# Zhengjun-Du/LC-CRF-SLAM

Hardware: AMD Instinct MI355X
Metric: CRF mean-field iters/sec (higher is better)
Workload: dtype f32; 1 GPU; C2: 2000 keypoints, 5 iters, two 2-D kernels (TUM3.yaml), L=2; frames_in_flight_per_gpu=16384, handles=1, distinct_frames=64, n_points=2000, n_iters=5, n_labels=2, engine=fused

## Files before the change

### lc-crf-slam_amd/csrc/engine.h

```cpp
#pragma once

#include <hip/hip_runtime.h>
#include <stdint.h>

#include <stdlib.h>

#include "../../include/lccrf.h"

#ifndef LCCRF_INSTRUMENT
#define LCCRF_INSTRUMENT 0
#endif

namespace lccrf {

#if LCCRF_INSTRUMENT
inline const char *ab_env(const char *name) { return getenv(name); }
#else
inline const char *ab_env(const char *) { return nullptr; }
#endif

constexpr int kMaxD = LCCRF_MAX_DIMS;
constexpr int kEmpty = -1;

constexpr int kNdistAxes = 4;
// ... 177 lines not shown
    c.nontemporal = c.alone_32bit > 0 && p.nontemporal;
    return p;
}

constexpr int kSortPlan = 3 * kMaxD + 2;
struct SortScratch {
    int bits;
    int rm_points;
    int *cells;
    int *partial;
    int *plan;
    int *code;
    int *hist;
    int *start;
    int *tiles;
    int *perm, *iperm;
    int vcap;
    int vbits;
    unsigned long long *vcode;
    unsigned long long *vkey;
    int *vph;
    int *vbad;
    int *vhist, *vstart;
    int *vtiles;
    int *vpartial;
    long long *vplan;
};

void launch_sort_points(const KernelDev &kd, const CrfDev &c, const SortScratch &ss, hipStream_t s);
void launch_permute_rows(const CrfDev &c, float *dst, const float *src, int width, int gather, hipStream_t s);
void launch_build_kernel(const KernelDev &kd, const CrfDev &c, hipStream_t s, const SortScratch *vsort, int *bstat);
void launch_norm(const KernelDev &kd, const CrfDev &c, int maxV, hipStream_t s);
struct UnaryTable { float v[2 * LCCRF_MAX_LABELS + 1]; };
void launch_unary_from_label_tbl(const CrfDev &c, const int16_t *label, const UnaryTable &tbl, hipStream_t s);
void launch_start(const CrfDev &c, hipStream_t s);
void launch_step_stream(const CrfDev &c, const KernelDev *kds, const int *maxV, float relax,
                        hipStream_t s, const float *const *compat = nullptr, const float *const *pre = nullptr);
void launch_norm_factor(const CrfDev &c, const float *norm, float *out, int root, hipStream_t s);
void launch_splat_scaled(const KernelDev &kd, const float *in, int in_stride, int L, int F, int maxV, const float *pre, hipStream_t s);
void launch_map(const CrfDev &c, hipStream_t s);
void launch_map_of(const CrfDev &c, const float *prob, int16_t *map, hipStream_t s);
void launch_exp_and_normalize(const CrfDev &c, const float *in, float *out, float scale, float relax, hipStream_t s);
void launch_step_init(const CrfDev &c, float *out, hipStream_t s);
void launch_filter(const KernelDev &kd, const CrfDev &c, int maxV, const float *in, float *out, int accumulate, hipStream_t s,
                   int reverse = 0, const float **blurred = nullptr, const float *compat = nullptr, const float *pre = nullptr);
const float *launch_filter_values1(const KernelDev &kd, const CrfDev &c, int maxV, const float *in, int in_stride, hipStream_t s,
                                   int reverse);
hipError_t time_blur_pass(const KernelDev &kd, int F, int maxV, int L, int reps, hipStream_t s, float *ms_per_launch);
enum { kStageCopy = 0, kStagePosition = 1, kStageImageU8 = 2, kStageImageF32 = 3 };
void launch_stage_features(float *dst, const void *src, int n, int d, int mode, int width, float posdev, float featuredev,
                           hipStream_t s);
void launch_validate_npoints(const int *in, int *out, int F, int maxN, int *bad, hipStream_t s);

struct BackwardRequest {
    int T;
    float relax;
    const float *grad_prob;
    float *grad_unary;
    float *grad_weights;
    float *const *grad_features;
    float *grad_compat;
    bool compat_form;
    float *grad_model;
    const int *counts;
};
struct BackwardArea {
    size_t slice;
// ... 54 lines not shown
inline int copy_matrices(const TermModel &t, int K, float (*mu)[4])
{
    int has_mu = 0;
    for (int k = 0; k < K; ++k)
        if (t.mats && t.mats[k]) {
            has_mu |= 1 << k;
            for (int e = 0; e < 4; ++e) mu[k][e] = t.mats[k][e];
        }
    return has_mu;
}
struct ConvergeOut {
    int *iterations;
    float *delta;
    int *changed;
    int *converged;
};

bool build_small_supported(const KernelDev *kds, int n, int max_points);
void launch_build_small(const KernelDev *kds, int n, int max_points, const CrfDev &c, hipStream_t s);

bool slam_shaped(const CrfDev &c, const KernelDev *kds, bool u16_tables);
bool fused_supported(const CrfDev &c, const KernelDev *kds, const int *maxV, const int *maxRow,
                     size_t *lds_bytes);
struct LeanPrep {
    unsigned char *buf = nullptr;
    size_t bytes = 0;
    bool valid = false, timed = false;
    unsigned long long key = 0, seen_key = 0;
    unsigned runs = 0;
    hipEvent_t ev0 = nullptr, ev1 = nullptr;
};
size_t lean_prep_bytes(const CrfDev &c, const KernelDev *kds, const int *maxV, const int *maxRow);
inline int fused_report(int lanes, int ppt, int chain0) { return lanes | ppt << 16 | (chain0 ? 1 << 20 : 0); }
struct SizedRequest {
    Schedule run;
    TermModel terms;
    ConvergeOut out;
    LeanPrep *prep;
};
struct SizedLaunch {
    int report;
    int shape;
};
SizedLaunch launch_inference(const CrfDev &c, const KernelDev *kds, const int *maxV, const int *maxRow, const SizedRequest &rq,
                             hipStream_t s);

struct ConvergeTrack {
    float *prev;
    unsigned *acc;
    int *done;
    int *running;
    ConvergeOut out;
};
void launch_track_begin(const CrfDev &c, const ConvergeTrack &tk, int max_iter, hipStream_t s);
void launch_track_step(const CrfDev &c, const ConvergeTrack &tk, int t, int max_iter, int criterion, float tol, hipStream_t s);
void launch_track_restore(const CrfDev &c, const ConvergeTrack &tk, int t_last, hipStream_t s);

bool frame_supported(const CrfDev &c, const KernelDev *kds);
struct FrameRequest {
    Schedule run;
    TermModel terms;
    int *status;
    int *frame_status;
    const int16_t *label;
    const float *tbl5;
    unsigned *done;
    unsigned done_epoch;
    ConvergeOut out;
    bool allow_small;
    unsigned *dual;
    unsigned dual_epoch;
// ... 24 lines not shown
```

### lc-crf-slam_amd/csrc/fused_engine.hip

```cpp
#include "engine.h"
#include "device_math.h"
#include "fused_loop.h"
#include "fused_lean.h"
#include "fused_variant.h"
#include "dispatch.h"

#include <algorithm>
#include <cstdio>
#include <cstdlib>

namespace lccrf {

namespace {

using namespace fl;

constexpr int kPrepMinFrames = 64;

struct FusedArgs {
    KernelDev kd[kMaxFusedK];
    FusedLayout lay;
    int n_iter, with_map;
    float relax, omr;
    long long *timing;
    int timing_block, timing_lane;
    int dbg;
    unsigned char *prep;
    int prep_stride;
    int Vcap[kMaxFusedK];
};

template <int NT, int PPT, int K, int CH, int MODE>
__global__ void __launch_bounds__(NT, 4) k_fused(CrfDev c, FusedArgs a)
{
    constexpr int D1 = kD1;
    extern __shared__ __attribute__((aligned(16))) unsigned char smem[];
    const int f = blockIdx.x;
// ... 503 lines not shown
    for (int k = 0; k < c.K; ++k) a.Vcap[k] = maxV[k];
    const LeanPrepPlan pp = lean_prep_plan(a.lay, c.K, a.Vcap, sh.nt, sh.ppt, sh.lean);
    static const bool no_prep = ab_env("LCCRF_NO_LEAN_PREP") != nullptr;
    int mode = 0;
    const int pieces = (sh.lean ? 1 : 2) * sh.nt * 16;
    bool pieces_ok = true;
    for (int k = 0; k < c.K; ++k) pieces_ok = pieces_ok && pp.row_bytes[k] <= pieces && pp.nbr_bytes[k] <= pieces;
    if (prep && prep->buf && !no_prep && pieces_ok && c.F >= kPrepMinFrames && (size_t)pp.total * (size_t)c.F <= prep->bytes) {
        unsigned long long key = 1469598103934665603ull;
        auto mix = [&](const void *p, size_t n) { for (size_t i = 0; i < n; ++i) key = (key ^ static_cast<const unsigned char *>(p)[i]) * 1099511628211ull; };
        mix(&a.lay, sizeof(a.lay));
        mix(a.Vcap, sizeof(int) * c.K);
        const int shape[6] = {c.F, c.K, sh.ppt, sh.points, sh.nt, sh.lean ? 2 : sh.small ? 1 : 0};
        mix(shape, sizeof(shape));
        mix(&kLeanPrepFormat, sizeof(kLeanPrepFormat));
        mix(&pp, sizeof(pp));
        a.prep = prep->buf;
        a.prep_stride = pp.total;
        if (prep->valid && prep->key == key) {
            mode = 2;
        } else if (prep->seen_key == key) {
            if (prep->ev0) (void)hipEventRecord(prep->ev0, s);
            launch_shape(c, a, s, 1, sh);
            if (prep->ev1) (void)hipEventRecord(prep->ev1, s);
            prep->timed = prep->ev0 && prep->ev1;
            prep->valid = true;
            prep->key = key;
            ++prep->runs;
            mode = 2;
        } else {
            prep->seen_key = key;
        }
    }
    launch_shape(c, a, s, mode, sh);
    stamps.print(s);
    return SizedLaunch{fused_report(sh.nt, sh.ppt, a.lay.chain0), sh.report()};
}

}
```

### lc-crf-slam_amd/csrc/fused_lean.h

```cpp
#pragma once

#include "fused_loop.h"

#ifndef LCCRF_LEAN_SKIP
#define LCCRF_LEAN_SKIP 0
#endif
#define LEAN_SKIP(bit) ((LCCRF_LEAN_SKIP & (bit)) != 0)

namespace lccrf {
namespace fl {

#ifndef LCCRF_CHAIN_TOP
#define LCCRF_CHAIN_TOP 16
#endif
constexpr int kLeanChainTop = LCCRF_CHAIN_TOP;
static_assert(kLeanChainTop == kChainTop || kLeanChainTop == 32, "16 rows on the lanes chain_top_rank names, or a full wavefront");
constexpr int kLeanMaxRounds = 4;
__host__ __device__ constexpr int lean_rounds(int nt) { return nt >= 512 ? 3 : 4; }
__host__ __device__ constexpr int lean_max_v(int nt) { return 3 * (nt - 64); }

__host__ __device__ inline int lean_plane_floats(int NA, int V0)
{
    const int top = V0 < kLeanChainTop ? V0 : kLeanChainTop;
    return (NA * kD1 + 11 * top + 3 * (V0 - top) + 16 + 63) & ~63;
// ... 390 lines not shown
    }
    for (int j = 0; j < kD1; ++j) {
        for (int v = tid; v < Vk; v += NT) {
            const unsigned n = gnbr[(size_t)j * Epad + v], n1 = n & 0xffffu, n2 = n >> 16;
            out[j * axis_words + perm[v]] = (n1 ? (unsigned)perm[n1 - 1] + 1u : 0u) | ((n2 ? (unsigned)perm[n2 - 1] + 1u : 0u) << 16);
        }
    }
    __syncthreads();
    for (int v = tid; v <= Vk; v += NT) row[v] = nrow[v];
    __syncthreads();
}

typedef unsigned lean_u3 __attribute__((ext_vector_type(3)));
struct LeanSrc {
    __amdgpu_buffer_rsrc_t nbr[kMaxFusedK];
    __amdgpu_buffer_rsrc_t bary[kMaxFusedK];
    __amdgpu_buffer_rsrc_t norm[kMaxFusedK];
    __amdgpu_buffer_rsrc_t unary;
    int nbr_axis_bytes[kMaxFusedK];
    int off_nbr[kMaxFusedK], off_bary[kMaxFusedK], off_norm[kMaxFusedK], off_unary;
};
constexpr int kLeanRecPoints = 4 * kNTSmall;
constexpr int kLeanRecUnary = 0;
constexpr int kLeanRecBary = kLeanRecUnary + kLeanRecPoints * 8;
constexpr int kLeanRecNorm = kLeanRecBary + kMaxFusedK * kLeanRecPoints * kD1 * 4;
constexpr int kLeanRecNbr = kLeanRecNorm + kMaxFusedK * kLeanRecPoints * 4;
constexpr int kLeanRecNbrAxis = lean_max_v(kNTSmall) * 4;
constexpr int kLeanRecBytes = (kLeanRecNbr + kD1 * kLeanRecNbrAxis + 255) & ~255;
__device__ __forceinline__ __amdgpu_buffer_rsrc_t lean_rsrc(const void *p, size_t bytes)
{
    return __builtin_amdgcn_make_buffer_rsrc(const_cast<void *>(p), 0, (int)bytes, 0x00020000);
}

template <int PPT, int K>
__device__ __forceinline__ void opaque_ids(PointRegs<PPT, K> &pr)
{
#pragma unroll
    for (int s = 0; s < PPT; ++s) {
#pragma unroll
        for (int k = 0; k < K; ++k) asm volatile("" : "+v"(pr.ix[s][k][0]), "+v"(pr.ix[s][k][1]), "+v"(pr.ix[s][k][2]));
    }
}

struct LeanPrepPlan {
    int cl_off;
    int row_off[kMaxFusedK], row_bytes[kMaxFusedK];
    int nbr_off[kMaxFusedK], nbr_bytes[kMaxFusedK];
    int snbr_off[kMaxFusedK], snbr_axis[kMaxFusedK];
    int total;
};
constexpr unsigned kLeanPrepFormat = 8;
__host__ __device__ inline LeanPrepPlan lean_prep_plan(const FusedLayout &lay, int K, const int *Vcap, int nt, int ppt, bool sorted = false)
{
    LeanPrepPlan p{};
    int o = K * ppt * nt * 12;
    p.cl_off = o;
    o += nt * 8;
    for (int k = 0; k < K; ++k) {
        p.row_off[k] = o;
        p.row_bytes[k] = ((Vcap[k] + 2) * 2 + 15) & ~15;
        o += p.row_bytes[k];
        p.nbr_off[k] = o;
        p.nbr_bytes[k] = lay.nbr[k] >= 0 ? ((kD1 * Vcap[k] * 4 + 15) & ~15) : 0;
        o += p.nbr_bytes[k];
    }
    for (int k = 0; k < K; ++k) {
        p.snbr_off[k] = o;
        p.snbr_axis[k] = (sorted && lay.nbr[k] < 0) ? ((Vcap[k] + 3) & ~3) * 4 : 0;
        o += kD1 * p.snbr_axis[k];
    }
    p.total = (o + 255) & ~255;
    return p;
}

template <int PPT, int K, int CH, int NT, bool RELOAD, bool NORM = false, bool PRELOADED = false>
__device__ __forceinline__ void mean_field_lean(unsigned char *smem, const FusedLayout &lay, const int (&V)[K], int N, int &t,
                                                PointRegs<PPT, K> &pr, ChainLane &cl, const float (&alpha)[K],
                                                const float (&wk)[K], const LeanSrc &src, int n_iter, float relax, float omr, Instr &ins)
{
    constexpr int D1 = kD1;
    constexpr int KF = K - 1;
    const int wave_base = __builtin_amdgcn_readfirstlane(t & ~63);
    (void)wave_base;
#define LEAN_FRESH_T()                                                                                               \
    do {                                                                                                             \
        int z_ = 0;                                                                                                  \
        asm volatile("" : "+v"(z_));                                                                                 \
        t = wave_base + (int)__builtin_amdgcn_mbcnt_hi(~0u, __builtin_amdgcn_mbcnt_lo(~0u, (unsigned)z_));          \
    } while (0)
    auto load_weights = [&]() {
        if (!RELOAD) return;
#pragma unroll
        for (int s = 0; s < PPT; ++s) {
            const int i = t + s * NT;
            if (!NORM) {
                typedef unsigned lean_u2 __attribute__((ext_vector_type(2)));
                const lean_u2 u = __builtin_amdgcn_raw_buffer_load_b64(src.unary, i * 8, src.off_unary, 0);
                pr.un[s] = make_float2(__uint_as_float(u.x), __uint_as_float(u.y));
            }
#pragma unroll
            for (int k = 0; k < K; ++k) {
                const lean_u3 b = __builtin_amdgcn_raw_buffer_load_b96(src.bary[k], i * (D1 * 4), src.off_bary[k], 0);
                pr.bary[s][k][0] = __uint_as_float(b.x);
                pr.bary[s][k][1] = __uint_as_float(b.y);
                pr.bary[s][k][2] = __uint_as_float(b.z);
                if (!NORM) pr.wn[s][k] = __uint_as_float(__builtin_amdgcn_raw_buffer_load_b32(src.norm[k], i * 4, src.off_norm[k], 0));
            }
        }
        if (NORM) return;
#pragma unroll
        for (int s = 0; s < PPT; ++s)
#pragma unroll
            for (int k = 0; k < K; ++k) pr.wn[s][k] = wk[k] * pr.wn[s][k];
    };
    auto phase_P = [&](int k) {
#pragma unroll
        for (int s = 0; s < PPT; ++s)
            if (t + s * NT < N) point_products_lean<PPT, K, CH>(lay, pr, s, k);
        if (chain_k<CH>(lay, k)) chain_pads_lean(smem, cl, t);
    };
    auto phase_S = [&](int k) {
        float *val = reinterpret_cast<float *>(smem + lay.val[k][0]);
        if (chain_k<CH>(lay, k)) {
            const int nwaves = lean_chain_waves(V[k]);
            if (__builtin_expect((t >> 6) < nwaves, 1)) {
                FL_PSTAMP();
                if ((t >> 6) == 0) __builtin_amdgcn_s_setprio(3);
                asm volatile("" : "+v"(cl.a), "+v"(cl.b));
// ... 121 lines not shown
        const float2 *src_v = reinterpret_cast<const float2 *>(smem + lay.val[k][j & 1]);
        float2 *dst = reinterpret_cast<float2 *>(smem + lay.val[k][(j & 1) ^ 1]);
#pragma unroll
        for (int r = 0; r < RA; ++r) {
            if (r < rounds) {
                const int v = lane + r * stride;
                if (v < V[k]) blur_vertex(src_v, dst, v, w[r]);
            }
        }
    };
    auto blur_small = [&](int lane, int j_lo, int j_hi) {
        const unsigned *tbl = reinterpret_cast<const unsigned *>(smem + lay.nbr[0]);
#pragma unroll
        for (int j = 0; j < D1; ++j) {
            if (j < j_lo || j >= j_hi) continue;
            const float2 *src_v = reinterpret_cast<const float2 *>(smem + lay.val[0][j & 1]);
            float2 *dst = reinterpret_cast<float2 *>(smem + lay.val[0][(j & 1) ^ 1]);
            for (int v = lane; v < V[0]; v += 64) blur_vertex(src_v, dst, v, tbl[j * V[0] + v]);
            asm volatile("s_waitcnt lgkmcnt(0)" ::: "memory");
            __builtin_amdgcn_wave_barrier();
        }
    };
    auto point_update = [&](int s) {
        if constexpr (NORM) {
#pragma unroll
            for (int k = 0; k < K; ++k) {
                const float v = slice_point_lean(pr, s, k, alpha[k]).x;
                const float nrm = 1.0f / (v + 1e-20f);
                if (RELOAD) __builtin_amdgcn_raw_buffer_store_b32(__float_as_uint(nrm), src.norm[k], (t + s * NT) * 4, src.off_norm[k], 0);
                else pr.wn[s][k] = wk[k] * nrm;
            }
            return;
        }
        float nx[2] = {-pr.un[s].x, -pr.un[s].y};
#pragma unroll
        for (int k = 0; k < K; ++k) {
            const float2 t = slice_point_lean(pr, s, k, alpha[k]);
            nx[0] += pr.wn[s][k] * t.x;
            nx[1] += pr.wn[s][k] * t.y;
        }
        pr.q[s] = softmax2(nx[0], nx[1], pr.q[s], relax, omr);
    };

    if (n_iter <= 0) return;
    if (!PRELOADED) load_weights();
#pragma unroll
    for (int s = 0; s < PPT; ++s)
        if (t + s * NT < N) point_products_lean<PPT, K, CH>(lay, pr, s, KF);
    if (chain_k<CH>(lay, KF)) chain_pads_lean(smem, cl, t);
    for (int it = 0; it < n_iter; ++it) {
        LEAN_FRESH_T();
        if (RELOAD) opaque_ids(pr);
        else opaque(pr);
        unsigned w[OVL ? 1 : K][D1][R];
        unsigned wa[RA], wb[2][RB];
        if constexpr (OVL) load_nbr_ovl(wa, wb);
        else load_nbr(w);
        __syncthreads();
        FL_STAMP();
        phase_S(KF);
#pragma unroll
        for (int k = KF - 1; k >= 0; --k) {
            __syncthreads();
            opaque_ids(pr);
            phase_P(k);
            __syncthreads();
            phase_S(k);
// ... 45 lines not shown
```

### lc-crf-slam_amd/csrc/host_engine.h

```cpp
#pragma once

#include "engine.h"

#include <vector>

namespace lccrf {

int fail(int code, const char *fmt, ...);
bool default_single_wg(), default_frame_general();

#define HIP_TRY(expr)                                                                        \
    do {                                                                                     \
        hipError_t e_ = (expr);                                                              \
        if (e_ != hipSuccess)                                                                \
            return fail(e_ == hipErrorOutOfMemory ? LCCRF_E_NOMEM : LCCRF_E_HIP, "%s: %s",  \
                        #expr, hipGetErrorString(e_));                                       \
    } while (0)

inline void cpu_relax()
{
#if defined(__x86_64__) || defined(__i386__)
    __builtin_ia32_pause();
#elif defined(__aarch64__)
    asm volatile("yield" ::: "memory");
// ... 62 lines not shown
    int activeN = 0;
    CrfDev crf{};
    int *npoints_own = nullptr;
    float *unary_own = nullptr;
    int16_t *label_own = nullptr;
    hipEvent_t ev_order = nullptr;
    int *npoints_bad = nullptr;
    float *io_a = nullptr, *io_b = nullptr;
    int16_t *io_map = nullptr;
    bool unary_set = false, built = false, sizes_known = false, started = false;

    int *V_host = nullptr;
    int *row_host = nullptr;
    size_t row_stride() const { return (size_t)Fcap * (1 + kBuildStats); }
    int *long_host = nullptr;
    std::vector<KernelState> kernels;
    std::vector<KernelState> spare;
    std::vector<KernelDev> kdevs;
    std::vector<int> maxV, maxRow;
    int built_upto = 0;

    int engine_pref = 0;
    int sized_engine = 1;
    int last_with_map = 0;
    size_t fused_lds = 0;
    LeanPrep lean_prep;
    bool fused_fits = false;
    bool batch_owned = false;

    bool unary_deferred = false;
    const int16_t *deferred_label = nullptr;
    UnaryTable deferred_tbl{};
    bool unary_is_label = false;

    int *late_status = nullptr;
    bool late_ok = false;
    Schedule late{0, 0, 1.0f, false, 0, 0.0f};
    int (*after_rerun)(void *) = nullptr;
    void *after_rerun_ctx = nullptr;
    static constexpr int kDualMaxFrames = 64;
    unsigned *dual_area = nullptr;
    unsigned dual_epoch = 0;
    unsigned *done_word = nullptr;
    unsigned done_epoch = 0;
    int16_t *map_host = nullptr;
    enum class Flight {
        kUnknown,
        kPending,
        kPendingDone,
        kPendingLabels,
        kLabelsSeen,
        kDoneSeen,
        kParkedDoneDue,
    } flight = Flight::kUnknown;
    bool run_pending() const { return flight == Flight::kPending || flight == Flight::kPendingDone || flight == Flight::kPendingLabels; }
    void touched() { if (flight == Flight::kLabelsSeen || flight == Flight::kDoneSeen) flight = Flight::kUnknown; }
    void done_seen() { flight = Flight::kDoneSeen; }
    bool take_labels(int16_t *out, int n);

    int *frame_status = nullptr;
    int *frame_status_host = nullptr;
    int *fb_list = nullptr;
    int *fb_list_host = nullptr;
    Engine *fb = nullptr;
    bool frame_small_ok = true;
    bool frame_small_used = false;
// ... 177 lines not shown
```

### lc-crf-slam_amd/csrc/host_engine.hip

```cpp
#include "host_engine.h"

#include <cmath>
#include <algorithm>
#include <cstring>

namespace lccrf {

void Engine::free_backward_area()
{
    if (!bwd_area) return;
    if (stream) (void)hipStreamSynchronize(stream);
    (void)hipFree(bwd_area);
    bwd_area = nullptr;
    bwd_area_bytes = 0;
}

int Engine::ensure_backward_area(size_t need)
{
    if (need <= bwd_area_bytes) return LCCRF_OK;
    free_backward_area();
    void *p = nullptr;
    const hipError_t ea = hipMalloc(&p, need);
    if (ea != hipSuccess) {
        (void)hipGetLastError();
// ... 282 lines not shown
    if ((rc = mem.alloc(&k.csr_w, Fz * E))) return rc;
    if ((rc = mem.alloc(&k.csr_pos, Fz * E))) return rc;
    if ((rc = mem.alloc(&k.pk, Fz * E))) return rc;
    if ((rc = mem.alloc(&k.nbr16, Fz * k.D1 * E))) return rc;
    if ((rc = mem.alloc(&k.norm, Fz * maxN))) return rc;
    if ((rc = mem.alloc(&k.val0, Fz * k.vstride))) return rc;
    if ((rc = mem.alloc(&k.val1, Fz * k.vstride))) return rc;
    if (own_features) {
        if ((rc = mem.alloc(&ks.feat_own, Fz * maxN * d))) return rc;
        k.feat = ks.feat_own;
    }
    if (stage)
        if ((rc = mem.alloc_pinned(&ks.feat_stage, Fz * maxN * d))) return rc;
    ks.maxV = k.Epad;
    kernels.push_back(ks);
    sync_views();
    return LCCRF_OK;
}

void Engine::recycle()
{
    const bool due = stream && flight == Flight::kLabelsSeen;
    if (stream && !due && flight != Flight::kDoneSeen) (void)hipStreamSynchronize(stream);
    flight = due ? Flight::kParkedDoneDue : Flight::kUnknown;
    free_backward_area();
    for (auto &ks : kernels) spare.push_back(ks);
    kernels.clear();
    F = Fcap;
    crf.unary = unary_own;
    crf.n_points = npoints_own;
    forget_inputs();
    unary_deferred = false;
    perm_on = vorder_on = perm_banned = false;
    unary_is_label = unary_p_valid = false;
    engine_pref = 0;
    report = RunReport{};
    model.clear(*this);
    sync_views();
}

void Engine::sync_views()
{
    kdevs.resize(kernels.size());
    maxV.resize(kernels.size());
    maxRow.resize(kernels.size());
    for (size_t i = 0; i < kernels.size(); ++i) {
        kernels[i].dev.V_host = V_host + i * Fcap;
        kernels[i].dev.rowmax_host = row_host + i * row_stride();
        kernels[i].dev.perm = perm_on ? sort.perm : nullptr;
        kernels[i].dev.iperm = perm_on ? sort.iperm : nullptr;
        kernels[i].dev.vorder = (perm_on && vorder_on && sort.vkey && kernels[i].dev.Epad <= sort.vcap) ? 1 : 0;
        kdevs[i] = kernels[i].dev;
        maxV[i] = kernels[i].maxV;
        maxRow[i] = kernels[i].maxRow;
    }
    model.views_changed();
    crf.K = (int)kernels.size();
    crf.F = F;
    crf.activeN = activeN;
    crf.perm = perm_on ? sort.perm : nullptr;
    crf.perm_stride = maxNpad;
}

int Engine::build_kernels(int k0, int n, bool may_reorder)
{
    for (int k = k0; k < k0 + n; ++k) {
        kernels[k].maxV = kernels[k].dev.Epad;
        kernels[k].root_valid = false;
    }
    if (k0 == 0) {
        static const bool no_perm = ab_env("LCCRF_NO_PERM") != nullptr;
        const int NAp = active_points(crf);
        const bool want = allow_perm && !no_perm && !perm_banned && (!perm_scoped || may_reorder) && n > 0 && n == (int)kernels.size() && NAp >= perm_min_points();
        if (want || perm_on) {
            if (unary_is_label) unary_deferred = true;
            unary_p_valid = false;
        }
        perm_on = false;
        static const char *env_vo = ab_env("LCCRF_VERTEX_ORDER");
        const int vo = env_vo ? (atoi(env_vo) ? 1 : 2) : opt.vertex_order;
        vorder_on = want && !vorder_broken && vo != 2;
        sync_views();
        if (want) {
            int rcs = ensure_sort_scratch();
            if (rcs) return rcs;
            int src = 0;
            for (int k = 1; k < n; ++k)
                if (kernels[k].dev.d > kernels[src].dev.d) src = k;
            sort.rm_points = vorder_on ? 1 : 0;
            launch_sort_points(kdevs[src], crf, sort, stream);
            HIP_TRY(hipGetLastError());
            perm_on = true;
        }
    }
    sync_views();
    const bool no_small = ab_env("LCCRF_NO_FUSED_BUILD") != nullptr;
    int k = k0;
    while (k < k0 + n) {
        int m = 1;
        const int NA = active_points(crf);
        const bool small_ok = !no_small && !perm_on;
        if (small_ok && k + 1 < k0 + n && build_small_supported(&kdevs[k], 2, NA)) m = 2;
        if (small_ok && build_small_supported(&kdevs[k], m, NA)) {
            for (int u = 0; u < m; ++u) kernels[k + u].dev.nbr2_ok = kernels[k + u].dev.nbrc_ok = kernels[k + u].dev.fast0_ok = kernels[k + u].dev.longrow_ok = 0;
            for (int u = 0; u < m; ++u) kernels[k + u].build_counted = false;
            launch_build_small(&kdevs[k], m, NA, crf, stream);
        } else {
            m = 1;
            kernels[k].dev.nbr2_ok = kernels[k].dev.nbr2 != nullptr;
// ... 87 lines not shown
        const int NAr = active_points(crf);
        kd.long_mode = kd.longrow_ok && (nlong > 0 || (long)NAr * kd.D1 > 4L * std::max(m, 1));
        if (kd.long_mode && (long)NAr * kd.D1 >= 16L * std::max(m, 1)) kd.long_mode = 2;
        kernels[k].maxV = m;
        kernels[k].maxRow = r;
    }
    sync_views();
    sizes_known = true;
    invalidate_lean_prep();
    fused_fits = engine_pref != 1 && !perm_on && fused_supported(crf, kdevs.data(), maxV.data(), maxRow.data(), &fused_lds);
    choose_sized_engine();
    if (engine_pref == 2 && !fused_fits)
        return fail(LCCRF_E_CAPACITY, "fused engine requested but the problem does not fit one workgroup's LDS");
    return LCCRF_OK;
}

UnaryTable Engine::label_table(const float *conf) const
{
    UnaryTable tb;
    tb.v[0] = -logf(1.0f / L);
    for (int i = 0; i < L; ++i) {
        tb.v[1 + i] = -logf((1.0f - conf[i]) / (L - 1));
        tb.v[1 + L + i] = -logf(conf[i]);
    }
    return tb;
}

void Engine::defer_unary_from_label(const int16_t *label, const float *conf)
{
    const UnaryTable tb = label_table(conf);
    crf.unary = unary_own;
    unary_deferred = true;
    unary_is_label = true;
    deferred_label = label;
    deferred_tbl = tb;
    unary_set = true;
}

void Engine::bind_unary(const float *p)
{
    crf.unary = const_cast<float *>(p);
    unary_deferred = unary_is_label = unary_p_valid = false;
    unary_set = true;
}

int Engine::ensure_unary()
{
    if (!unary_deferred) return LCCRF_OK;
    unary_deferred = false;
    launch_unary_from_label_tbl(crf, deferred_label, deferred_tbl, stream);
    HIP_TRY(hipGetLastError());
    return LCCRF_OK;
}

int Engine::start()
{
    if (!unary_set) return fail(LCCRF_E_STATE, "unary energies not set");
    if (int rc = make_ready(kSettled | kCallerOrder | kUnaries)) return rc;
    launch_start(crf, stream);
    started = true;
    return LCCRF_OK;
}

int Engine::step(float relax)
{
    if (!started) return fail(LCCRF_E_STATE, "stepInference before startInference");
    const int rc = make_ready(kSettled | kCallerOrder | kSized | kUnaries | kStepViews);
    if (rc) return rc;
    launch_step_stream(crf, step_kdevs(), maxV.data(), relax, stream, model.compat_arg(), model.pre_arg());
    return LCCRF_OK;
}

bool Engine::frame_ok() const
{
    static const bool no_frame = ab_env("LCCRF_NO_FRAME") != nullptr;
    if (model.general() && !(opt.frame_general && L == 2 && active_points(crf) <= kGeneralMaxPoints)) return false;
    return !no_frame && engine_pref == 0 && !kernels.empty() && frame_supported(crf, kdevs.data());
}

int Engine::run_frame(const Schedule &run)
{
    const int with_map = run.with_map;
    const bool stop = run.until_converged;
    const bool general = model.general();
// ... 64 lines not shown
            invalidate_lattices();
            rc = flush_builds();
        }
    }
    if (!rc && (needs & kSized)) rc = learn_sizes(reorder);
    else if (!rc && (needs & kBuilt)) rc = flush_builds(reorder);
    if (!rc && (needs & kUnaries)) rc = ensure_unary();
    if (!rc && (needs & kStepViews)) rc = model.ensure_factors(*this);
    if (call_ban) perm_banned = false;
    return rc;
}

int Engine::run(int n_iter, int with_map, float relax)
{
    if (n_iter < 0) return fail(LCCRF_E_INVALID, "n_iterations < 0");
    if (!unary_set) return fail(LCCRF_E_STATE, "unary energies not set");
    int rc = resolve_late();
    if (rc) return rc;
    if (frame_ok()) return run_frame(fixed_run(n_iter, with_map, relax));
    invalidate_lattices();
    return inference_sized(fixed_run(n_iter, with_map, relax));
}

int Engine::engine_in_use(int *out)
{
    const bool hbm = built && report.engine != 3;
    if (int rc = hbm ? make_ready(kSized) : LCCRF_OK) return rc;
    *out = report.in_use(hbm ? sized_engine : 0);
    return LCCRF_OK;
}

bool Engine::launch_sized(const Schedule &run, LeanPrep *prep)
{
    const SizedRequest rq{run, model.terms(kernels.size()), conv_out(), prep};
    const SizedLaunch r = launch_inference(crf, step_kdevs(), maxV.data(), maxRow.data(), rq, stream);
    if (!r.report) return false;
    report.sized_run(sized_engine, r, run.until_converged, rq.terms.general());
    started = true;
    if (run.until_converged) conv_valid = true;
    return true;
}

int Engine::inference_sized(const Schedule &run, unsigned more_needs)
{
    const int rc = make_ready(kSized | kUnaries | kStepViews | more_needs);
    if (rc) return rc;
    report.ran_on(sized_engine, false);
    last_with_map = run.with_map;
    if (perm_on || sized_engine == 1) {
        const CrfDev v = begin_iteration();
        for (int it = 0; it < run.n_iter; ++it) launch_step_stream(v, step_kdevs(), maxV.data(), run.relax, stream, model.compat_arg(), model.pre_arg());
        end_iteration(run.with_map);
        HIP_TRY(hipGetLastError());
        return LCCRF_OK;
    }
    const size_t prep_need = sized_engine == 2 ? lean_prep_bytes(crf, kdevs.data(), maxV.data(), maxRow.data()) : 0;
    if (prep_need > lean_prep.bytes) {
        lean_prep.valid = false;
        lean_prep.buf = nullptr;
        lean_prep.bytes = 0;
        unsigned char *p = nullptr;
        if (mem.alloc(&p, prep_need, false) == LCCRF_OK) {
            lean_prep.buf = p;
            lean_prep.bytes = prep_need;
        } else {
            (void)hipGetLastError();
        }
// ... 108 lines not shown
```

### lc-crf-slam_amd/csrc/stream_pointwise.hip

```cpp
#include "stream_common.h"
#include "device_math.h"
#include <algorithm>

namespace lccrf {
namespace {

__global__ void __launch_bounds__(kBlock) k_unary_from_label_tbl(CrfDev c, const int16_t *__restrict__ label, UnaryTable tbl)
{
    const int f = blockIdx.y;
    const int idx = blockIdx.x * kBlock + threadIdx.x;
    if (idx >= c.n_points[f] * c.L) return;
    const int i = idx / c.L, m = idx - i * c.L;
    const int t = label[(size_t)f * c.maxN + (c.perm ? c.perm[(size_t)f * c.perm_stride + i] : i)];
    float u;
    if (t < 0 || t >= c.L) u = tbl.v[0];
    else u = (m == t) ? tbl.v[1 + c.L + t] : tbl.v[1 + t];
    c.unary[((size_t)f * c.maxN + i) * c.L + m] = u;
}

__global__ void __launch_bounds__(kBlock) k_softmax(CrfDev c, const float *__restrict__ in,
                                                    float *__restrict__ out, float scale, float relax)
{
    const int f = blockIdx.y;
    const int i = blockIdx.x * kBlock + threadIdx.x;
    if (i >= c.n_points[f]) return;
    const size_t q = ((size_t)f * c.maxN + i) * c.L;
    exp_and_normalize_row(in + q, out + q, c.L, scale, relax);
}

constexpr int kSoftmaxMaxL = 32;
__global__ void __launch_bounds__(kBlock) k_softmax_rows(CrfDev c, const float *__restrict__ in, float *__restrict__ out, float scale, float relax)
{
    const int f = blockIdx.y, L = c.L;
    const int N = c.n_points[f];
    const int rpw = 64 / L;
    const int lane = threadIdx.x & 63, wave = blockIdx.x * (kBlock / 64) + (threadIdx.x >> 6);
    const int row = lane / L, j = lane - row * L, i = wave * rpw + row;
    const bool live = row < rpw && i < N;
    const size_t q = ((size_t)f * c.maxN + (live ? i : 0)) * L + (live ? j : 0);
    const float s = live ? scale * in[q] : 0.0f;
    const int first = row * L;
    float mx = __shfl(s, first, 64);
    for (int t0 = 1; t0 < L; t0 += 8) {
        float v[8];
#pragma unroll
        for (int u = 0; u < 8; ++u) v[u] = __shfl(s, first + min(t0 + u, L - 1), 64);
#pragma unroll
        for (int u = 0; u < 8; ++u)
            if (t0 + u < L && mx < v[u]) mx = v[u];
    }
// ... 21 lines not shown
    const size_t q = (size_t)f * c.maxN * c.L + idx;
    out[q] = -c.unary[q];
}

__global__ void __launch_bounds__(kBlock) k_map(CrfDev c, const float *__restrict__ Q, int16_t *__restrict__ map)
{
    const int f = blockIdx.y;
    const int i = blockIdx.x * kBlock + threadIdx.x;
    const int N = c.n_points[f];
    int lab = 0;
    if (i < N) {
        const float *p = Q + ((size_t)f * c.maxN + i) * c.L;
        lab = argmax_row(p, c.L);
        map[(size_t)f * c.maxN + i] = (int16_t)lab;
    }
    if (c.map_bits && map == c.map && c.L == 2 && (i >> 6) < c.bits_stride) {
        const unsigned long long m = __ballot(lab == 1);
        if ((threadIdx.x & 63) == 0) c.map_bits[(size_t)f * c.bits_stride + (i >> 6)] = m;
    }
}

__global__ void __launch_bounds__(kBlock) k_validate_npoints(const int *__restrict__ in, int *__restrict__ out, int F,
                                                             int maxN, int *bad)
{
    const int f = blockIdx.x * kBlock + threadIdx.x;
    if (f >= F) return;
    const int n = in[f], c = min(max(n, 0), maxN);
    out[f] = c;
    if (c != n) *bad = 1;
}

}

void launch_unary_from_label_tbl(const CrfDev &c, const int16_t *label, const UnaryTable &tbl, hipStream_t s)
{
    k_unary_from_label_tbl<<<grid_for((long)c.maxN * c.L, c.F), kBlock, 0, s>>>(c, label, tbl);
}

void launch_exp_and_normalize(const CrfDev &c, const float *in, float *out, float scale, float relax, hipStream_t s)
{
    if (c.L >= 3 && c.L <= kSoftmaxMaxL) {
        const int per_block = (kBlock / 64) * (64 / c.L);
        k_softmax_rows<<<dim3((unsigned)((c.maxN + per_block - 1) / per_block), (unsigned)c.F), kBlock, 0, s>>>(c, in, out, scale, relax);
    } else {
        k_softmax<<<grid_for(c.maxN, c.F), kBlock, 0, s>>>(c, in, out, scale, relax);
    }
}

void launch_start(const CrfDev &c, hipStream_t s) { launch_exp_and_normalize(c, c.unary, c.Q, -1.0f, 1.0f, s); }

void launch_validate_npoints(const int *in, int *out, int F, int maxN, int *bad, hipStream_t s)
{
    k_validate_npoints<<<(F + kBlock - 1) / kBlock, kBlock, 0, s>>>(in, out, F, maxN, bad);
}

void launch_map(const CrfDev &c, hipStream_t s) { launch_map_of(c, c.Q, c.map, s); }

void launch_map_of(const CrfDev &c, const float *prob, int16_t *map, hipStream_t s)
{
    k_map<<<grid_for(c.maxN, c.F), kBlock, 0, s>>>(c, prob, map);
}

void launch_step_init(const CrfDev &c, float *out, hipStream_t s)
{
    k_step_init<<<grid_for((long)c.maxN * c.L, c.F), kBlock, 0, s>>>(c, out);
}

template <typename T>
__global__ void __launch_bounds__(kBlock) k_copy_frames(T *__restrict__ dst, size_t dst_stride, const T *__restrict__ src,
// ... 44 lines not shown
```

Before: 50.69 million iters/s.

## Feed lean fused kernel byte label codes instead of float unary pairs

When the unary comes from a two-label table, the unary kernel now also writes a one-byte code per point plus a tiny 12-float table of the three possible negated unaries and their initial softmax. A new lean fused kernel variant reads these codes, reconstructs each point's unary and initial Q by selection from registers, and skips the per-point 8-byte unary load and softmax initialisation. This reduces global memory traffic per frame, at the cost of an extra kernel instantiation, an extra small allocation, and more state to invalidate when permutation or unary binding changes.

```diff
diff --git a/lc-crf-slam_amd/csrc/engine.h b/lc-crf-slam_amd/csrc/engine.h
--- a/lc-crf-slam_amd/csrc/engine.h
+++ b/lc-crf-slam_amd/csrc/engine.h
@@ -233,7 +233,8 @@
 void launch_build_kernel(const KernelDev &kd, const CrfDev &c, hipStream_t s, const SortScratch *vsort, int *bstat);
 void launch_norm(const KernelDev &kd, const CrfDev &c, int maxV, hipStream_t s);
 struct UnaryTable { float v[2 * LCCRF_MAX_LABELS + 1]; };
-void launch_unary_from_label_tbl(const CrfDev &c, const int16_t *label, const UnaryTable &tbl, hipStream_t s);
+void launch_unary_from_label_tbl(const CrfDev &c, const int16_t *label, const UnaryTable &tbl, hipStream_t s,
+                                 unsigned char *codes = nullptr, float *pairs = nullptr);
 void launch_start(const CrfDev &c, hipStream_t s);
 void launch_step_stream(const CrfDev &c, const KernelDev *kds, const int *maxV, float relax,
                         hipStream_t s, const float *const *compat = nullptr, const float *const *pre = nullptr);
@@ -354,11 +355,17 @@
 };
 size_t lean_prep_bytes(const CrfDev &c, const KernelDev *kds, const int *maxV, const int *maxRow);
 inline int fused_report(int lanes, int ppt, int chain0) { return lanes | ppt << 16 | (chain0 ? 1 << 20 : 0); }
+constexpr int kLabelPairFloats = 12;
+struct LabelCodes {
+    const unsigned char *codes;
+    const float *pairs;
+};
 struct SizedRequest {
     Schedule run;
     TermModel terms;
     ConvergeOut out;
     LeanPrep *prep;
+    LabelCodes lbl;
 };
 struct SizedLaunch {
     int report;
diff --git a/lc-crf-slam_amd/csrc/fused_engine.hip b/lc-crf-slam_amd/csrc/fused_engine.hip
--- a/lc-crf-slam_amd/csrc/fused_engine.hip
+++ b/lc-crf-slam_amd/csrc/fused_engine.hip
@@ -3,6 +3,7 @@
 #include "fused_loop.h"
 #include "fused_lean.h"
 #include "fused_variant.h"
+#include "fused_lean_label.h"
 #include "dispatch.h"
 
 #include <algorithm>
@@ -572,7 +573,28 @@
             prep->seen_key = key;
         }
     }
-    launch_shape(c, a, s, mode, sh);
+    if (mode == 2 && sh.lean && rq.lbl.codes && rq.lbl.pairs && !ab_env("LCCRF_NO_LABEL_CODES")) {
+        LeanLabelArgs la{};
+        for (int k = 0; k < c.K; ++k) {
+            la.kd[k] = a.kd[k];
+            la.Vcap[k] = a.Vcap[k];
+        }
+        la.lay = a.lay;
+        la.n_iter = a.n_iter;
+        la.with_map = a.with_map;
+        la.relax = a.relax;
+        la.omr = a.omr;
+        la.timing = a.timing;
+        la.timing_block = a.timing_block;
+        la.timing_lane = a.timing_lane;
+        la.dbg = a.dbg;
+        la.prep = a.prep;
+        la.prep_stride = a.prep_stride;
+        la.lbl = rq.lbl;
+        launch_lean_label(c, la, sh.ppt, s);
+    } else {
+        launch_shape(c, a, s, mode, sh);
+    }
     stamps.print(s);
     return SizedLaunch{fused_report(sh.nt, sh.ppt, a.lay.chain0), sh.report()};
 }
diff --git a/lc-crf-slam_amd/csrc/fused_lean.h b/lc-crf-slam_amd/csrc/fused_lean.h
--- a/lc-crf-slam_amd/csrc/fused_lean.h
+++ b/lc-crf-slam_amd/csrc/fused_lean.h
@@ -446,6 +446,15 @@
     return __builtin_amdgcn_make_buffer_rsrc(const_cast<void *>(p), 0, (int)bytes, 0x00020000);
 }
 
+struct LeanLabel {
+    unsigned codes;
+    float n0x, n0y, n1x, n1y, n2x, n2y;
+};
+__device__ __forceinline__ float lean_pick(unsigned code, float v0, float v1, float v2)
+{
+    return code == 0 ? v0 : code == 1 ? v1 : v2;
+}
+
 template <int PPT, int K>
 __device__ __forceinline__ void opaque_ids(PointRegs<PPT, K> &pr)
 {
@@ -487,10 +496,11 @@
     return p;
 }
 
-template <int PPT, int K, int CH, int NT, bool RELOAD, bool NORM = false, bool PRELOADED = false>
+template <int PPT, int K, int CH, int NT, bool RELOAD, bool NORM = false, bool PRELOADED = false, bool LBL = false>
 __device__ __forceinline__ void mean_field_lean(unsigned char *smem, const FusedLayout &lay, const int (&V)[K], int N, int &t,
                                                 PointRegs<PPT, K> &pr, ChainLane &cl, const float (&alpha)[K],
-                                                const float (&wk)[K], const LeanSrc &src, int n_iter, float relax, float omr, Instr &ins)
+                                                const float (&wk)[K], const LeanSrc &src, int n_iter, float relax, float omr, Instr &ins,
+                                                const LeanLabel &lb = LeanLabel{})
 {
     constexpr int D1 = kD1;
     constexpr int KF = K - 1;
@@ -507,7 +517,7 @@
 #pragma unroll
         for (int s = 0; s < PPT; ++s) {
             const int i = t + s * NT;
-            if (!NORM) {
+            if (!NORM && !LBL) {
                 typedef unsigned lean_u2 __attribute__((ext_vector_type(2)));
                 const lean_u2 u = __builtin_amdgcn_raw_buffer_load_b64(src.unary, i * 8, src.off_unary, 0);
                 pr.un[s] = make_float2(__uint_as_float(u.x), __uint_as_float(u.y));
@@ -695,7 +705,15 @@
             }
             return;
         }
-        float nx[2] = {-pr.un[s].x, -pr.un[s].y};
+        float nx[2];
+        if constexpr (LBL) {
+            const unsigned code = (lb.codes >> (8 * s)) & 0xffu;
+            nx[0] = lean_pick(code, lb.n0x, lb.n1x, lb.n2x);
+            nx[1] = lean_pick(code, lb.n0y, lb.n1y, lb.n2y);
+        } else {
+            nx[0] = -pr.un[s].x;
+            nx[1] = -pr.un[s].y;
+        }
 #pragma unroll
         for (int k = 0; k < K; ++k) {
             const float2 t = slice_point_lean(pr, s, k, alpha[k]);
diff --git a/lc-crf-slam_amd/csrc/fused_lean_label.h b/lc-crf-slam_amd/csrc/fused_lean_label.h
--- /dev/null
+++ b/lc-crf-slam_amd/csrc/fused_lean_label.h
@@ -0,0 +1,22 @@
+#pragma once
+
+#include "fused_loop.h"
+
+namespace lccrf {
+
+struct LeanLabelArgs {
+    KernelDev kd[fl::kMaxFusedK];
+    fl::FusedLayout lay;
+    int n_iter, with_map;
+    float relax, omr;
+    long long *timing;
+    int timing_block, timing_lane;
+    int dbg;
+    unsigned char *prep;
+    int prep_stride;
+    int Vcap[fl::kMaxFusedK];
+    LabelCodes lbl;
+};
+void launch_lean_label(const CrfDev &c, const LeanLabelArgs &a, int ppt, hipStream_t s);
+
+}
diff --git a/lc-crf-slam_amd/csrc/fused_lean_label.hip b/lc-crf-slam_amd/csrc/fused_lean_label.hip
--- /dev/null
+++ b/lc-crf-slam_amd/csrc/fused_lean_label.hip
@@ -0,0 +1,152 @@
+#include "engine.h"
+#include "device_math.h"
+#include "fused_loop.h"
+#include "fused_lean.h"
+#include "fused_lean_label.h"
+#include "dispatch.h"
+
+namespace lccrf {
+
+namespace {
+
+using namespace fl;
+
+template <int NT, int PPT, int K, int CH, bool RELOAD>
+__global__ void __launch_bounds__(NT, 4) k_fused_lean_lbl(CrfDev c, LeanLabelArgs a)
+{
+    constexpr int D1 = kD1;
+    static_assert(PPT <= 4, "a lane's codes share one register");
+    extern __shared__ __attribute__((aligned(16))) unsigned char smem[];
+    const int f = blockIdx.x;
+    const int tid = threadIdx.x;
+    const int N = c.n_points[f];
+    Instr ins{a.timing, a.timing_block, a.dbg, 0, a.timing_lane};
+    FL_STAMP();
+
+    PointRegs<PPT, K> pr;
+    int V[K];
+#pragma unroll
+    for (int k = 0; k < K; ++k) V[k] = a.kd[k].V[f];
+    const int wave_base = __builtin_amdgcn_readfirstlane(tid & ~63);
+    auto lane_id = [&]() {
+        int z = 0;
+        asm volatile("" : "+v"(z));
+        return wave_base + (int)__builtin_amdgcn_mbcnt_hi(~0u, __builtin_amdgcn_mbcnt_lo(~0u, (unsigned)z));
+    };
+    const FusedLayout &lay = a.lay;
+    float wk[K];
+    LeanSrc src;
+#pragma unroll
+    for (int k = 0; k < K; ++k) {
+        const KernelDev &kd = a.kd[k];
+        wk[k] = kd.w;
+        src.nbr[k] = lean_rsrc(kd.nbr16 + (size_t)f * D1 * kd.Epad, (size_t)D1 * kd.Epad * 4);
+        src.bary[k] = lean_rsrc(kd.bary + (size_t)f * kd.Epad, (size_t)kd.Epad * 4);
+        src.norm[k] = lean_rsrc(kd.norm + (size_t)f * kd.maxN, (size_t)kd.maxN * 4);
+        src.nbr_axis_bytes[k] = kd.Epad * 4;
+        src.off_nbr[k] = src.off_bary[k] = src.off_norm[k] = 0;
+    }
+    src.unary = src.norm[0];
+    src.off_unary = 0;
+    const LeanPrepPlan pp = lean_prep_plan(lay, K, a.Vcap, NT, PPT, true);
+    const __amdgpu_buffer_rsrc_t rp = lean_rsrc(a.prep + (size_t)f * a.prep_stride, (size_t)a.prep_stride);
+    const __amdgpu_buffer_rsrc_t rc = lean_rsrc(a.lbl.codes + (size_t)f * c.maxN, (size_t)c.maxN);
+#pragma unroll
+    for (int k = 0; k < K; ++k) {
+        if (!chain_k<CH>(lay, k)) {
+            src.nbr[k] = lean_rsrc(a.prep + (size_t)f * a.prep_stride + pp.snbr_off[k], (size_t)D1 * pp.snbr_axis[k]);
+            src.nbr_axis_bytes[k] = pp.snbr_axis[k];
+        }
+    }
+    typedef unsigned lean_u2 __attribute__((ext_vector_type(2)));
+    typedef unsigned lean_u4 __attribute__((ext_vector_type(4)));
+    LeanLabel lb;
+    const float *const tb = a.lbl.pairs;
+    lb.n0x = tb[0], lb.n0y = tb[1], lb.n1x = tb[2], lb.n1y = tb[3], lb.n2x = tb[4], lb.n2y = tb[5];
+    const float q0x = tb[6], q0y = tb[7], q1x = tb[8], q1y = tb[9], q2x = tb[10], q2y = tb[11];
+    unsigned code[PPT];
+#pragma unroll
+    for (int s = 0; s < PPT; ++s) {
+        code[s] = __builtin_amdgcn_raw_buffer_load_b8(rc, tid + s * NT, 0, 0);
+#pragma unroll
+        for (int k = 0; k < K; ++k) {
+            const lean_u3 w = __builtin_amdgcn_raw_buffer_load_b96(rp, tid * 12, ((s * K + k) * NT) * 12, 0);
+            pr.ix[s][k][0] = w.x;
+            pr.ix[s][k][1] = w.y;
+            pr.ix[s][k][2] = w.z;
+            const lean_u3 b = __builtin_amdgcn_raw_buffer_load_b96(src.bary[k], (tid + s * NT) * (D1 * 4), 0, 0);
+            pr.bary[s][k][0] = __uint_as_float(b.x);
+            pr.bary[s][k][1] = __uint_as_float(b.y);
+            pr.bary[s][k][2] = __uint_as_float(b.z);
+            pr.wn[s][k] = RELOAD ? 0.0f : __uint_as_float(__builtin_amdgcn_raw_buffer_load_b32(src.norm[k], (tid + s * NT) * 4, 0, 0));
+        }
+    }
+    const lean_u2 clw = __builtin_amdgcn_raw_buffer_load_b64(rp, tid * 8, pp.cl_off, 0);
+    lean_u4 trow[K], tnbr[K];
+#pragma unroll
+    for (int k = 0; k < K; ++k) {
+        trow[k] = tnbr[k] = lean_u4{0u, 0u, 0u, 0u};
+        if (tid * 16 < pp.row_bytes[k]) trow[k] = __builtin_amdgcn_raw_buffer_load_b128(rp, tid * 16, pp.row_off[k], 0);
+        if (tid * 16 < pp.nbr_bytes[k]) tnbr[k] = __builtin_amdgcn_raw_buffer_load_b128(rp, tid * 16, pp.nbr_off[k], 0);
+    }
+    FL_PSTAMP();
+    if (N <= 0) {
+        if (a.with_map) clear_label_bits<NT>(c, f, 0, lane_id());
+        return;
+    }
+#pragma unroll
+    for (int k = 0; k < K; ++k) {
+        if (tid * 16 < pp.row_bytes[k]) *reinterpret_cast<lean_u4 *>(smem + lay.row[k] + tid * 16) = trow[k];
+        if (tid * 16 < pp.nbr_bytes[k]) *reinterpret_cast<lean_u4 *>(smem + lay.nbr[k] + tid * 16) = tnbr[k];
+    }
+    if (tid < 32) reinterpret_cast<float *>(smem + lay.zero)[tid] = 0.0f;
+    if (tid == 0) {
+#pragma unroll
+        for (int k = 0; k < K; ++k) {
+            reinterpret_cast<float2 *>(smem + lay.val[k][0])[0] = make_float2(0.f, 0.f);
+            reinterpret_cast<float2 *>(smem + lay.val[k][1])[0] = make_float2(0.f, 0.f);
+        }
+    }
+#pragma unroll
+    for (int s = 0; s < PPT; ++s)
+#pragma unroll
+        for (int k = 0; k < K; ++k) pr.wn[s][k] = wk[k] * pr.wn[s][k];
+    lb.codes = 0;
+#pragma unroll
+    for (int s = 0; s < PPT; ++s) {
+        pr.un[s] = make_float2(0.f, 0.f);
+        pr.q[s] = make_float2(0.f, 0.f);
+        if (tid + s * NT < N) pr.q[s] = make_float2(lean_pick(code[s], q0x, q1x, q2x), lean_pick(code[s], q0y, q1y, q2y));
+        lb.codes |= code[s] << (8 * s);
+    }
+    FL_PSTAMP();
+    __syncthreads();
+    FL_PSTAMP();
+    ChainLane cl{clw.x, clw.y};
+    FL_STAMP();
+    float alpha[K];
+#pragma unroll
+    for (int k = 0; k < K; ++k) alpha[k] = a.kd[k].alpha;
+    int t = lane_id();
+    mean_field_lean<PPT, K, CH, NT, RELOAD, false, true, true>(smem, lay, V, N, t, pr, cl, alpha, wk, src, a.n_iter, a.relax, a.omr, ins, lb);
+    t = lane_id();
+    store_results<PPT, K, NT>(c, f, N, t, pr, a.with_map);
+    FL_STAMP();
+    if (kInstr && a.timing && (int)blockIdx.x == a.timing_block && t == a.timing_lane) a.timing[63] = ins.n;
+}
+
+}
+
+void launch_lean_label(const CrfDev &c, const LeanLabelArgs &a, int ppt, hipStream_t s)
+{
+    with_dims<1, kMaxFusedK>(c.K, [&](auto kk) {
+        with_dims<0, 1>(a.lay.chain0 ? 1 : 0, [&](auto ch) {
+            with_dims<1, 4>(ppt, [&](auto p) {
+                constexpr int K = decltype(kk)::value, CH = decltype(ch)::value, P = decltype(p)::value;
+                launch_workgroups(k_fused_lean_lbl<kNTSmall, P, K, CH, (P >= 3)>, c.F, kNTSmall, a.lay.total, s, c, a);
+            });
+        });
+    });
+}
+
+}
diff --git a/lc-crf-slam_amd/csrc/host_engine.h b/lc-crf-slam_amd/csrc/host_engine.h
--- a/lc-crf-slam_amd/csrc/host_engine.h
+++ b/lc-crf-slam_amd/csrc/host_engine.h
@@ -118,6 +118,9 @@
     const int16_t *deferred_label = nullptr;
     UnaryTable deferred_tbl{};
     bool unary_is_label = false;
+    unsigned char *label_codes = nullptr;
+    float *label_pairs = nullptr;
+    bool label_codes_valid = false;
 
     int *late_status = nullptr;
     bool late_ok = false;
diff --git a/lc-crf-slam_amd/csrc/host_engine.hip b/lc-crf-slam_amd/csrc/host_engine.hip
--- a/lc-crf-slam_amd/csrc/host_engine.hip
+++ b/lc-crf-slam_amd/csrc/host_engine.hip
@@ -338,7 +338,7 @@
     forget_inputs();
     unary_deferred = false;
     perm_on = vorder_on = perm_banned = false;
-    unary_is_label = unary_p_valid = false;
+    unary_is_label = unary_p_valid = label_codes_valid = false;
     engine_pref = 0;
     report = RunReport{};
     model.clear(*this);
@@ -380,7 +380,7 @@
         const bool want = allow_perm && !no_perm && !perm_banned && (!perm_scoped || may_reorder) && n > 0 && n == (int)kernels.size() && NAp >= perm_min_points();
         if (want || perm_on) {
             if (unary_is_label) unary_deferred = true;
-            unary_p_valid = false;
+            unary_p_valid = label_codes_valid = false;
         }
         perm_on = false;
         static const char *env_vo = ab_env("LCCRF_VERTEX_ORDER");
@@ -534,6 +534,7 @@
     crf.unary = unary_own;
     unary_deferred = true;
     unary_is_label = true;
+    label_codes_valid = false;
     deferred_label = label;
     deferred_tbl = tb;
     unary_set = true;
@@ -542,7 +543,7 @@
 void Engine::bind_unary(const float *p)
 {
     crf.unary = const_cast<float *>(p);
-    unary_deferred = unary_is_label = unary_p_valid = false;
+    unary_deferred = unary_is_label = unary_p_valid = label_codes_valid = false;
     unary_set = true;
 }
 
@@ -550,8 +551,21 @@
 {
     if (!unary_deferred) return LCCRF_OK;
     unary_deferred = false;
-    launch_unary_from_label_tbl(crf, deferred_label, deferred_tbl, stream);
+    label_codes_valid = false;
+    if (L == 2 && !label_codes) {
+        unsigned char *pc = nullptr;
+        float *pp = nullptr;
+        if (mem.alloc(&pc, (size_t)Fcap * maxN, false) == LCCRF_OK && mem.alloc(&pp, (size_t)kLabelPairFloats) == LCCRF_OK) {
+            label_codes = pc;
+            label_pairs = pp;
+        } else {
+            (void)hipGetLastError();
+        }
+    }
+    const bool lbl = L == 2 && label_codes && crf.unary == unary_own;
+    launch_unary_from_label_tbl(crf, deferred_label, deferred_tbl, stream, lbl ? label_codes : nullptr, lbl ? label_pairs : nullptr);
     HIP_TRY(hipGetLastError());
+    label_codes_valid = lbl;
     return LCCRF_OK;
 }
 
@@ -682,7 +696,9 @@
 
 bool Engine::launch_sized(const Schedule &run, LeanPrep *prep)
 {
-    const SizedRequest rq{run, model.terms(kernels.size()), conv_out(), prep};
+    const bool lbl = label_codes_valid && unary_is_label && !unary_deferred && !perm_on && crf.unary == unary_own;
+    const SizedRequest rq{run, model.terms(kernels.size()), conv_out(), prep,
+                          LabelCodes{lbl ? label_codes : nullptr, lbl ? label_pairs : nullptr}};
     const SizedLaunch r = launch_inference(crf, step_kdevs(), maxV.data(), maxRow.data(), rq, stream);
     if (!r.report) return false;
     report.sized_run(sized_engine, r, run.until_converged, rq.terms.general());
diff --git a/lc-crf-slam_amd/csrc/stream_pointwise.hip b/lc-crf-slam_amd/csrc/stream_pointwise.hip
--- a/lc-crf-slam_amd/csrc/stream_pointwise.hip
+++ b/lc-crf-slam_amd/csrc/stream_pointwise.hip
@@ -5,10 +5,19 @@
 namespace lccrf {
 namespace {
 
-__global__ void __launch_bounds__(kBlock) k_unary_from_label_tbl(CrfDev c, const int16_t *__restrict__ label, UnaryTable tbl)
+__global__ void __launch_bounds__(kBlock) k_unary_from_label_tbl(CrfDev c, const int16_t *__restrict__ label, UnaryTable tbl,
+                                                                 unsigned char *__restrict__ codes, float *__restrict__ pairs)
 {
     const int f = blockIdx.y;
     const int idx = blockIdx.x * kBlock + threadIdx.x;
+    if (pairs && f == 0 && idx < 3) {
+        const float a = idx == 2 ? tbl.v[0] : idx == 0 ? tbl.v[3] : tbl.v[2], b = idx == 2 ? tbl.v[0] : idx == 0 ? tbl.v[1] : tbl.v[4];
+        const float2 q0 = softmax2_fresh(-a, -b);
+        pairs[2 * idx] = -a;
+        pairs[2 * idx + 1] = -b;
+        pairs[6 + 2 * idx] = q0.x;
+        pairs[6 + 2 * idx + 1] = q0.y;
+    }
     if (idx >= c.n_points[f] * c.L) return;
     const int i = idx / c.L, m = idx - i * c.L;
     const int t = label[(size_t)f * c.maxN + (c.perm ? c.perm[(size_t)f * c.perm_stride + i] : i)];
@@ -16,6 +25,7 @@
     if (t < 0 || t >= c.L) u = tbl.v[0];
     else u = (m == t) ? tbl.v[1 + c.L + t] : tbl.v[1 + t];
     c.unary[((size_t)f * c.maxN + i) * c.L + m] = u;
+    if (codes && m == 0) codes[(size_t)f * c.maxN + i] = (t < 0 || t >= c.L) ? 2 : (unsigned char)t;
 }
 
 __global__ void __launch_bounds__(kBlock) k_softmax(CrfDev c, const float *__restrict__ in,
@@ -103,9 +113,11 @@
 
 }
 
-void launch_unary_from_label_tbl(const CrfDev &c, const int16_t *label, const UnaryTable &tbl, hipStream_t s)
+void launch_unary_from_label_tbl(const CrfDev &c, const int16_t *label, const UnaryTable &tbl, hipStream_t s, unsigned char *codes,
+                                 float *pairs)
 {
-    k_unary_from_label_tbl<<<grid_for((long)c.maxN * c.L, c.F), kBlock, 0, s>>>(c, label, tbl);
+    const bool lbl = codes && pairs && c.L == 2;
+    k_unary_from_label_tbl<<<grid_for((long)c.maxN * c.L, c.F), kBlock, 0, s>>>(c, label, tbl, lbl ? codes : nullptr, lbl ? pairs : nullptr);
 }
 
 void launch_exp_and_normalize(const CrfDev &c, const float *in, float *out, float scale, float relax, hipStream_t s)
```

Measured after the change: 52.65 million iters/s, median of 6. +3.9%, better.
